# toandaominh1997/EfficientDet.Pytorch

Hardware: AMD Instinct MI355X
Metric: images/sec EfficientDet-D0 512px fwd+bwd (higher is better)
Workload: dtype f32_hf16x3_bwd_bf16x3

## Files before the change

efficientdet/pytorch_amd/_lib.py:

```python
import ctypes as C
import os

import torch

HERE = os.path.dirname(os.path.abspath(__file__))
LIB_PATH = os.environ.get('EFFDET_HIP_LIB') or os.path.join(os.path.dirname(os.path.abspath(__file__)), 'libeffdet_hip.so')
MAX_SEG = 5
MAX_CONV_SEG = 10
ABI_VERSION = 11
F32, BF16, F32_BF16X3, F32_SPLIT = 0, 1, 2, 3
F32_HSPLIT = 4
ACT_NONE, ACT_RELU, ACT_SWISH, ACT_SIGMOID = 0, 1, 2, 3
RES_NONE, RES_ADD, RES_RELU_MASK, RES_SWISH_GRAD = 0, 1, 2, 3
TUNE_IGEMM_BIG, TUNE_IGEMM_BIG_MIN_M, TUNE_SPLIT_PERS, TUNE_IGEMM_KORD, TUNE_SPLIT_KORD = 0, 1, 2, 3, 4
TUNE_ROWSLAB = 5

_ERR = {-1: 'EFFDET_EINVAL', -2: 'EFFDET_ELAUNCH', -3: 'EFFDET_EUNSUPPORTED'}


class Seg(C.Structure):
    _fields_ = [('H', C.c_int), ('W', C.c_int), ('Ho', C.c_int), ('Wo', C.c_int),
                ('in_off', C.c_longlong), ('in_bstride', C.c_longlong),
                ('out_off', C.c_longlong), ('out_bstride', C.c_longlong)]


class ConvDesc(C.Structure):
    _fields_ = [('x', C.c_void_p), ('w', C.c_void_p), ('y', C.c_void_p), ('z', C.c_void_p), ('res', C.c_void_p),
                ('scale', C.c_void_p), ('shift', C.c_void_p), ('rowscale', C.c_void_p),
                ('bc_scale', C.c_void_p), ('bc_shift', C.c_void_p),
                ('dtype', C.c_int), ('out_f32', C.c_int),
                ('B', C.c_int), ('Cin', C.c_int), ('Cout', C.c_int), ('KH', C.c_int), ('KW', C.c_int),
                ('stride', C.c_int), ('pad_t', C.c_int), ('pad_l', C.c_int),
                ('ldx', C.c_int), ('ldy', C.c_int), ('act', C.c_int), ('res_mode', C.c_int),
                ('nseg', C.c_int), ('seg', Seg * MAX_CONV_SEG), ('w_image_stride', C.c_longlong), ('y_split', C.c_void_p), ('range_flag', C.c_void_p),
                ('seg_w', C.c_void_p * MAX_CONV_SEG), ('seg_shift', C.c_void_p * MAX_CONV_SEG)]


class WgradDesc(C.Structure):
    _fields_ = [('x', C.c_void_p), ('dz', C.c_void_p), ('dw', C.c_void_p), ('dbias', C.c_void_p),
                ('dtype', C.c_int),
                ('B', C.c_int), ('Cin', C.c_int), ('Cout', C.c_int), ('KH', C.c_int), ('KW', C.c_int),
                ('stride', C.c_int), ('pad_t', C.c_int), ('pad_l', C.c_int),
                ('ldx', C.c_int), ('lddz', C.c_int), ('nseg', C.c_int), ('image_splits', C.c_int), ('seg', Seg * MAX_SEG)]


class PrepJob(C.Structure):
    _fields_ = [('a', C.c_void_p), ('b', C.c_void_p), ('c', C.c_void_p), ('d', C.c_void_p), ('out', C.c_void_p),
                ('kind', C.c_int), ('dtype', C.c_int), ('n0', C.c_int), ('n1', C.c_int), ('n2', C.c_int), ('n3', C.c_int),
                ('n4', C.c_int), ('eps', C.c_float)]


class UnpackJob(C.Structure):
    _fields_ = [(n, C.c_void_p) for n in ('g', 'scale', 'w_oihw', 'dw_oihw', 'wsum', 'dsum_part', 'mean', 'invstd', 'dgamma', 'dbeta',
                                          'dbias_out', 'slab_scale', 'slab_cscale')] + \
               [(n, C.c_int) for n in ('accumulate', 'Cout', 'Cin', 'KH', 'KW', 'Cin_pad', 'nslabs', 'slabs_per_scale')]


class SeParamJob(C.Structure):
    _fields_ = [(n, C.c_void_p) for n in ('du', 'dmid', 'sw', 'pool', 'dw1', 'db1', 'dw2', 'db2')] + \
               [('B', C.c_int), ('C', C.c_int), ('Cse', C.c_int), ('inv_hw', C.c_float)]


class DwUnpackJob(C.Structure):
    _fields_ = [(n, C.c_void_p) for n in ('g_kkc', 'scale', 'w_c1kk', 'dw_c1kk', 'wsum', 'dsum', 'mean', 'invstd', 'dgamma', 'dbeta')] + \
               [('C', C.c_int), ('kk', C.c_int)]


class _TailUnion(C.Union):
# ... 381 lines not shown
```

efficientdet/pytorch_amd/csrc/conv_igemm.hip:

```cpp
#include "common.h"
#include "../../../include/effdet_live_tiles.h"
#include "../../../include/effdet_needed_tiles.h"
#include "../../../include/effdet_unit_lists.h"
#include "../../../include/effdet_conv_plan.h"
#include "../../../include/effdet_gate_operand.h"
#include <stdlib.h>

#ifndef EFFDET_IGEMM_BIG_DEFAULT
#define EFFDET_IGEMM_BIG_DEFAULT 1
#endif

namespace {

struct SegD {
  int H, W, Ho, Wo, M, tile_start;
  long long in_off, in_bs, out_off, out_bs;
  unsigned x_bytes;
  long long w_off;
  long long sh_off;
};

struct ConvK {
  const void* x; const void* w; void* y; void* z; const void* res;
  const float* scale; const float* shift; const float* rowscale;
  const float* bc_scale; const float* bc_shift;
  int Cin, Cout, KW, stride, pad_t, pad_l;
  int ldx, ldy;
  int Kc;
  int cpt;
  int act, res_mode, out_f32, vec_ok;
  int out_split;
  int* range_flag;
  void* ysplit;
  int nseg, mtiles, ntiles;
  unsigned w_bytes;
  int kord;
  long long w_img_bytes;
  const unsigned char* live;
  int live_tile0;
  const unsigned char* needed;
  int needed_tile0;
  const unsigned char* uflags32; const int* units; const int* ucounts;
  long long g_in_off; unsigned g_x_bytes;
  const float* a_gate;
  int slab;
  int xld;
  SegD seg[EFFDET_MAX_CONV_SEG];
};

constexpr int BM = 128;

__host__ __device__ inline int slab_entries(int W) { return (BM / W) * (W + 2); }
__host__ __device__ inline bool slab_seg_ok(const SegD& s, int bn) {
  return (s.W & (s.W - 1)) == 0 && s.W >= (bn > 64 ? 8 : 16) && s.W <= 64 && s.Ho == s.H && s.Wo == s.W;
}
typedef float f32x16 __attribute__((ext_vector_type(16)));

template <typename T> struct Mma;
template <> struct Mma<bf16_t> {
  static __device__ __forceinline__ void run(const uint4& a, const uint4& b, f32x4& c) {
    c = __builtin_amdgcn_mfma_f32_16x16x32_bf16(__builtin_bit_cast(bf16x8, a), __builtin_bit_cast(bf16x8, b), c, 0, 0, 0);
  }
};
struct MmaH {
  static __device__ __forceinline__ void run(const uint4& a, const uint4& b, f32x4& c) {
    c = __builtin_amdgcn_mfma_f32_16x16x32_f16(__builtin_bit_cast(f16x8, a), __builtin_bit_cast(f16x8, b), c, 0, 0, 0);
  }
};
template <> struct Mma<float> {
  static __device__ __forceinline__ void run(const uint4& a, const uint4& b, f32x4& c) {
    c = __builtin_amdgcn_mfma_f32_16x16x4f32(__uint_as_float(a.x), __uint_as_float(b.x), c, 0, 0, 0);
    c = __builtin_amdgcn_mfma_f32_16x16x4f32(__uint_as_float(a.y), __uint_as_float(b.y), c, 0, 0, 0);
    c = __builtin_amdgcn_mfma_f32_16x16x4f32(__uint_as_float(a.z), __uint_as_float(b.z), c, 0, 0, 0);
    c = __builtin_amdgcn_mfma_f32_16x16x4f32(__uint_as_float(a.w), __uint_as_float(b.w), c, 0, 0, 0);
  }
};

template <typename T, int BN, int WAVES_N, int NWAVES, int SPLIT = 0, int NS = 2, int M32 = 0, int GATE = 0>
__global__ __launch_bounds__(NWAVES * 64, (SPLIT == 3 && NWAVES == 4) ? 3 : 1) void conv_igemm_kernel(const ConvK p) {
  static_assert(!SPLIT || sizeof(T) == 4, "bf16x3 splitting applies to fp32 storage");
  static_assert(!M32 || SPLIT == 2, "the 32x32x16 form is built for the split layout");
  static_assert(SPLIT != 3 || NS == 2, "f16x3: two stages");
  static_assert(NS == 2 || !M32, "deep staging is not built for the 32x32 tile loop");
  static_assert(!GATE || (SPLIT == 0 && sizeof(T) == 4), "the operand gate is built for the exact-fp32 form");
  constexpr int CE = Elem<T>::CE;
  constexpr int NTHREADS = NWAVES * 64;
  constexpr int WAVES_M = NWAVES / WAVES_N;
  constexpr int WTM = BM / WAVES_M, WTN = BN / WAVES_N;
  constexpr int MT = WTM / 16, NT = WTN / 16;
  constexpr int XLD = BM * 8;
  constexpr int WLD = BN * 8;
  constexpr int RSTEP = NTHREADS / 8;
  constexpr int XROWS = BM / RSTEP;
  constexpr int WROWS = (BN + RSTEP - 1) / RSTEP;

  constexpr bool SLABCAP = SPLIT >= 2 && NS == 2 && !M32;
  constexpr int SP = SLABCAP ? (160 + RSTEP - 1) / RSTEP : 1;
  static_assert(!SLABCAP || ((SP - 1) * RSTEP == 128 && WROWS * RSTEP == BN), "slab passes: 128 entries for every wave, the rest in the last pass");
  static_assert(!SLABCAP || MT <= 2, "slab fragments: fragment 1 is one uniform entry step from fragment 0");

  extern __shared__ __attribute__((aligned(16))) uint4 smem[];
  const int xld = SLABCAP ? p.xld : XLD;
  uint4* xs = SLABCAP ? smem + NS * WLD : smem;
  uint4* ws = SLABCAP ? smem : smem + NS * XLD;

  const int tid = threadIdx.x;
  const int lane = tid & 63, wave = tid >> 6;
  const int wm0 = (wave / WAVES_N) * WTM, wn0 = (wave % WAVES_N) * WTN;

  int tile = xcd_remap(blockIdx.x, gridDim.x);
  if constexpr (SPLIT == 2) {
    if (p.live) {
      const int b = blockIdx.x, whole = (p.mtiles >> 3) << 3;
      if (b < whole * p.ntiles) {
        const int i = b >> 3, j = i / p.ntiles;
        tile = (j * 8 + (b & 7)) * p.ntiles + (i - j * p.ntiles);
      } else tile = b;
    }
  }
  if constexpr (SPLIT == 3) {
    if (p.needed) {
      const int b = blockIdx.x, whole = (p.mtiles >> 3) << 3;
      if (b < whole * p.ntiles) {
        const int i = b >> 3, j = i / p.ntiles;
        tile = (j * 8 + (b & 7)) * p.ntiles + (i - j * p.ntiles);
      } else tile = b;
    }
  }
  const int mt = tile / p.ntiles, nt = tile - mt * p.ntiles;
  int si = 0;
#pragma unroll
  for (int s = 1; s < EFFDET_MAX_CONV_SEG; ++s)
    if (s < p.nseg && mt >= p.seg[s].tile_start) si = s;
  const SegD sg = p.seg[si];
  const int m_base = (mt - sg.tile_start) * BM;
  const int n_base = nt * BN;
  const int HoWo = sg.Ho * sg.Wo;
// ... 139 lines not shown
#pragma unroll
    for (int j = 0; j < WROWS; ++j) {
      if (wrow0 + RSTEP * j < BN)
        dma16_async(rw, ws_a + (unsigned)(buf * WLD + (wrow0 + RSTEP * j) * 8) * 16u, (kok && wok[j]) ? woff[j] + (unsigned)kq * 16u : EFFDET_OOB);
    }
    if constexpr (SPLIT != 1) {
      if (p.kord == 1) {
        const int taps = p.Kc / p.cpt;
        ++tapi;
        if (++kw == p.KW) { kw = 0; ++kh; }
        if (tapi == taps) { tapi = 0; kh = 0; kw = 0; cc += 8; }
        kq = (cc < p.cpt) ? tapi * p.cpt + cc : p.Kc;
        retap();
        return;
      }
    }
    kq += 8; cc += 8;
    if (cc < p.cpt) {
#pragma unroll
      for (int j = 0; j < XROWS; ++j) xcur[j] = (xcur[j] == EFFDET_OOB) ? EFFDET_OOB : xcur[j] + 128u;
    } else {
      while (cc >= p.cpt) { cc -= p.cpt; ++kw; if (kw == p.KW) { kw = 0; ++kh; } }
      retap();
    }
  };

  f32x4 acc[NT][MT];
#pragma unroll
  for (int a = 0; a < NT; ++a)
#pragma unroll
    for (int b = 0; b < MT; ++b) acc[a][b] = f32x4{0.f, 0.f, 0.f, 0.f};

  const int nk = (p.Kc + 7) >> 3;
  const int l15 = lane & 15, lq = lane >> 4, lsw = l15 >> 1;
  float* const gl = (float*)(smem + NS * (XLD + WLD));
  if constexpr (GATE) {
    const float* grow = p.a_gate + (long long)(m_base / HoWo) * p.Cin;
    for (int i = tid; i < nk * 32; i += NTHREADS) gl[i] = i < p.Cin ? grow[i] : 0.f;
  }
  auto load = [&](int buf, int s, uint4 (&wf)[NT], uint4 (&xf)[MT]) {
    const int ch = ((s * 4 + lq) ^ lsw);
#pragma unroll
    for (int a = 0; a < NT; ++a) wf[a] = ws[buf * WLD + (wn0 + a * 16 + l15) * 8 + ch];
#pragma unroll
    for (int b = 0; b < MT; ++b) xf[b] = xs[buf * XLD + (wm0 + b * 16 + l15) * 8 + ch];
  };
  auto mma = [&](const uint4 (&wf)[NT], const uint4 (&xf)[MT]) {
#pragma unroll
    for (int a = 0; a < NT; ++a)
#pragma unroll
      for (int b = 0; b < MT; ++b) Mma<T>::run(wf[a], xf[b], acc[a][b]);
  };
  constexpr int PPS = XROWS + WROWS;
  auto wait_tile = [&](int ahead) {
    if constexpr (NS == 2) { (void)ahead; dma_wait_all(); }
    else {
      if (NS >= 4 && ahead >= 2) asm volatile("s_waitcnt vmcnt(%0)" :: "n"(2 * PPS) : "memory");
      else if (ahead >= 1) asm volatile("s_waitcnt vmcnt(%0)" :: "n"(PPS) : "memory");
      else dma_wait_all();
    }
  };
  constexpr int NT32 = M32 ? WTN / 32 : 1, MT32 = M32 ? WTM / 32 : 1;
  f32x16 acc32[NT32][MT32];
  const int l31 = lane & 31, lh = lane >> 5;
  if constexpr (M32) {
    static_assert(WTN % 32 == 0 && WTM % 32 == 0, "32x32 MFMA tiles");
#pragma unroll
    for (int a = 0; a < NT32; ++a)
#pragma unroll
      for (int b = 0; b < MT32; ++b)
#pragma unroll
        for (int e = 0; e < 16; ++e) acc32[a][b][e] = 0.f;
    const int sw32 = (l31 >> 1) & 7;
    auto mm32 = [](const uint4& a, const uint4& b, f32x16& c) {
      c = __builtin_amdgcn_mfma_f32_32x32x16_bf16(__builtin_bit_cast(bf16x8, a), __builtin_bit_cast(bf16x8, b), c, 0, 0, 0);
    };
    auto kstep = [&](int buf) {
#pragma unroll
      for (int kk = 0; kk < 2; ++kk) {
        uint4 wh[NT32], wl[NT32], xh[MT32], xl[MT32];
        const int ch = ((2 * kk + lh) ^ sw32), cl = ((4 + 2 * kk + lh) ^ sw32);
#pragma unroll
        for (int a = 0; a < NT32; ++a) wh[a] = ws[buf * WLD + (wn0 + a * 32 + l31) * 8 + ch];
#pragma unroll
        for (int b = 0; b < MT32; ++b) xh[b] = xs[buf * XLD + (wm0 + b * 32 + l31) * 8 + ch];
#pragma unroll
        for (int b = 0; b < MT32; ++b) xl[b] = xs[buf * XLD + (wm0 + b * 32 + l31) * 8 + cl];
#pragma unroll
        for (int a = 0; a < NT32; ++a) wl[a] = ws[buf * WLD + (wn0 + a * 32 + l31) * 8 + cl];
#pragma unroll
        for (int t = 0; t < 3; ++t)
#pragma unroll
          for (int a = 0; a < NT32; ++a)
#pragma unroll
            for (int b = 0; b < MT32; ++b) mm32(t == 2 ? wl[a] : wh[a], t == 1 ? xl[b] : xh[b], acc32[a][b]);
      }
    };
    stage(0);
    if (nk > 1) stage(1);
    dma_wait_all();
    __syncthreads();
    for (int kt = 0; kt < nk; ++kt) {
      const int c = kt & 1;
      kstep(c);
      if (kt + 1 < nk) {
        dma_wait_all();
        __syncthreads();
        if (kt + 2 < nk) stage(c);
      }
    }
  } else if constexpr (SPLIT) {
    struct Frags { uint4 wh[NT], wl[NT], xh[MT], xl[MT]; };
    f32x4 acc2[SPLIT == 3 ? NT : 1][SPLIT == 3 ? MT : 1];
// ... 814 lines not shown
          const f32x4 xv = xt[cur][pl * C4 + k];
#pragma unroll
          for (int j = 0; j < 4; ++j) {
            const f32x2v xx = f32x2v{xv[j], xv[j]};
            a01 = __builtin_elementwise_fma(w01[4 * k + j], xx, a01);
            a23 = __builtin_elementwise_fma(w23[4 * k + j], xx, a23);
          }
        }
        f32x4 v = f32x4{a01[0], a01[1], a23[0], a23[1]} * sc + sh;
        if (p.z) *(f32x4*)((float*)p.z + o) = v;
        if (p.act == EFFDET_ACT_RELU) { for (int r = 0; r < 4; ++r) v[r] = relu_(v[r]); }
        else if (p.act == EFFDET_ACT_SWISH) { for (int r = 0; r < 4; ++r) v[r] = swishf_(v[r]); }
        else if (p.act == EFFDET_ACT_SIGMOID) { for (int r = 0; r < 4; ++r) v[r] = sigmoidf_(v[r]); }
        if (p.rowscale || p.bc_scale) {
          const int bi = m / HoWo;
          if (p.rowscale) v *= p.rowscale[bi];
          if (p.bc_scale) { const int bo = bi * p.Cout + n0; v = v * *(const f32x4*)(p.bc_scale + bo) + *(const f32x4*)(p.bc_shift + bo); }
        }
        if (p.res_mode == EFFDET_RES_ADD) { v += q; }
        else if (p.res_mode == EFFDET_RES_RELU_MASK) { for (int r = 0; r < 4; ++r) v[r] = relu_bwd_(q[r], v[r]); }
        else if (p.res_mode == EFFDET_RES_SWISH_GRAD) { for (int r = 0; r < 4; ++r) v[r] *= swish_gradf_(q[r]); }
        *(f32x4*)((float*)p.y + o) = v;
      }
    }
    if (tile + 1 < ntile) sstore(cur ^ 1);
    __syncthreads();
  }
}

static bool pw_eligible(const effdet_conv_t* p) {
  static const int on = getenv("EFFDET_CONV_PW") ? atoi(getenv("EFFDET_CONV_PW")) : 1;
  if (!on || p->dtype != EFFDET_F32 || p->out_f32 || p->nseg != 1 || p->KH != 1 || p->KW != 1 || p->stride != 1 || p->pad_t || p->pad_l) return false;
  if ((p->Cin != 16 && p->Cin != 24) || p->Cout % 4 || p->Cout < 32 || p->Cout > 1024) return false;
  const effdet_seg_t& g = p->seg[0];
  if (g.H != g.Ho || g.W != g.Wo || p->ldx != p->Cin || p->ldy != p->Cout) return false;
  if (g.in_bstride != (long long)g.H * g.W * p->ldx || g.out_bstride != (long long)g.Ho * g.Wo * p->ldy) return false;
  if (g.in_off % 4 || g.out_off % 4) return false;
  return (long long)p->B * g.H * g.W >= 65536;
}

struct ConvPlan {
  int id;
  ConvK k;
  int (*launch)(const ConvPlan&, hipStream_t);
  unsigned grid;
  size_t lds;
  int pw_G, pw_NPS, pw_ppw;
  int form, pers;
  int tile_m, tile_n, stages, threads, m32;
  int ksteps;
  int gate;
};

static int g_tuning[EFFDET_TUNE_COUNT] = {-1, 16384, -1, 1, -1, -1};
static bool rowslab_on() {
  if (g_tuning[EFFDET_TUNE_ROWSLAB] < 0) g_tuning[EFFDET_TUNE_ROWSLAB] = getenv("EFFDET_ROWSLAB") ? atoi(getenv("EFFDET_ROWSLAB")) : 1;
  return g_tuning[EFFDET_TUNE_ROWSLAB] != 0;
}

template <typename T, int BN, int WAVES_N, int NWAVES, int SPLIT, int NS, int M32, int GATE>
int launch_igemm(const ConvPlan& c, hipStream_t st) {
  if (c.lds > 48 * 1024) EFFDET_SET_MAX_LDS((conv_igemm_kernel<T, BN, WAVES_N, NWAVES, SPLIT, NS, M32, GATE>), c.lds);
  hipLaunchKernelGGL((conv_igemm_kernel<T, BN, WAVES_N, NWAVES, SPLIT, NS, M32, GATE>), dim3(c.grid), dim3(NWAVES * 64), c.lds, st, c.k);
  EFFDET_CHECK_LAUNCH();
  return EFFDET_OK;
}
template <typename T, int BN, int WAVES_N, int NWAVES, int SPLIT = 0, int NS = 2, int M32 = 0, int GATE = 0>
int use_igemm(ConvPlan& c, int id) {
  c.k.ntiles = (c.k.Cout + BN - 1) / BN;
  c.grid = (unsigned)(c.k.mtiles * c.k.ntiles);
  c.k.slab = 0; c.k.xld = BM * 8;
  if constexpr (SPLIT >= 2 && NS == 2 && !M32) {
    const ConvK& k = c.k;
    if (rowslab_on() && k.kord == 1 && k.KW == 3 && k.Kc == 9 * k.cpt && k.stride == 1 && k.pad_t == 1 && k.pad_l == 1) {
      int ent = 0;
      for (int s = 0; s < k.nseg; ++s)
        if (slab_seg_ok(k.seg[s], BN) && ((slab_entries(k.seg[s].W) + 7) & ~7) > ent) ent = (slab_entries(k.seg[s].W) + 7) & ~7;
      if (ent) { c.k.slab = 1; c.k.xld = (ent > BM ? ent : BM) * 8; }
    }
  }
  c.lds = (size_t)NS * (c.k.xld + BN * 8) * sizeof(uint4);
  if (GATE) c.lds += (size_t)((c.k.Kc + 7) >> 3) * 32 * sizeof(float);
  c.gate = GATE;
  c.launch = launch_igemm<T, BN, WAVES_N, NWAVES, SPLIT, NS, M32, GATE>;
  static_assert(EFFDET_CONV_FORM_PLAIN == 0 && EFFDET_CONV_FORM_BF16X3 == 1 && EFFDET_CONV_FORM_SPLIT == 2 && EFFDET_CONV_FORM_HSPLIT == 3,
                "the kernel's SPLIT parameter is the public form code");
  c.form = SPLIT; c.pers = 0; c.tile_m = BM; c.tile_n = BN; c.stages = NS; c.threads = NWAVES * 64; c.m32 = M32;
  c.ksteps = (c.k.Kc + 7) >> 3;
  return c.id = id;
}

template <int WM, int WN, int NS, int X3>
int launch_pers(const ConvPlan& c, hipStream_t st) {
  EFFDET_SET_MAX_LDS((conv_igemm_pers_kernel<WM, WN, NS, X3>), c.lds);
  static unsigned ncu = 0;
  if (ncu == 0) { int dev = 0; hipDeviceProp_t pr; ncu = (hipGetDevice(&dev) == hipSuccess && hipGetDeviceProperties(&pr, dev) == hipSuccess) ? pr.multiProcessorCount : 256; }
  const unsigned grid = c.grid < ncu ? c.grid : ncu;
  hipLaunchKernelGGL((conv_igemm_pers_kernel<WM, WN, NS, X3>), dim3(grid), dim3(WM * WN * 64), c.lds, st, c.k);
  EFFDET_CHECK_LAUNCH();
  return EFFDET_OK;
}
template <int WM, int WN, int NS, int X3 = 0>
int use_pers(ConvPlan& c, int id) {
  constexpr int TM = 64 * WM, TN = 64 * WN;
  ConvK& k = c.k;
  k.mtiles = 0;
  for (int s = 0; s < k.nseg; ++s) { k.seg[s].tile_start = k.mtiles; k.mtiles += (k.seg[s].M + TM - 1) / TM; }
  k.ntiles = (k.Cout + TN - 1) / TN;
  if (X3) {
    k.ldx *= 2;
    for (int s = 0; s < k.nseg; ++s) { k.seg[s].in_off *= 2; k.seg[s].in_bs *= 2; }
  }
  c.grid = (unsigned)(k.mtiles * k.ntiles);
  c.lds = (size_t)NS * (TM + TN) * 128;
  c.launch = launch_pers<WM, WN, NS, X3>;
  c.form = X3 ? EFFDET_CONV_FORM_SPLIT : EFFDET_CONV_FORM_PLAIN; c.pers = 1; c.tile_m = TM; c.tile_n = TN; c.stages = NS; c.threads = WM * WN * 64; c.m32 = 1;
  c.ksteps = (k.Kc / k.cpt) * (k.cpt >> 3);
  return c.id = id;
}
static int use_big(ConvPlan& c, int id) {
  switch (id) {
    case 10 + 442: return use_pers<4, 4, 2>(c, id);
    case 10 + 242: return use_pers<2, 4, 2>(c, id);
    case 10 + 243: return use_pers<2, 4, 3>(c, id);
    case 10 + 4220: return use_pers<4, 2, 2>(c, id);
    default: return use_pers<4, 2, 3>(c, id);
  }
}

template <int CIN>
int launch_pw(const ConvPlan& c, hipStream_t st) {
  hipLaunchKernelGGL(conv_pw_f32_kernel<CIN>, dim3(c.grid), dim3(256), 0, st, c.k, c.k.seg[0].M, c.pw_G, c.pw_NPS, c.pw_ppw);
  EFFDET_CHECK_LAUNCH();
  return EFFDET_OK;
}
static int use_pw(ConvPlan& c) {
  c.pw_G = c.k.Cout / 4; c.pw_NPS = 256 / c.pw_G; c.pw_ppw = 1024;
  c.grid = (unsigned)((c.k.seg[0].M + c.pw_ppw - 1) / c.pw_ppw);
  c.lds = 0;
  c.launch = c.k.Cin == 16 ? launch_pw<16> : launch_pw<24>;
  c.form = EFFDET_CONV_FORM_SKINNY; c.pers = 0; c.tile_m = 64; c.tile_n = c.k.Cout; c.stages = 2; c.threads = 256; c.m32 = 0;
  c.k.mtiles = (int)c.grid; c.k.ntiles = 1; c.ksteps = 1;
  return c.id = 20;
}

static int big_variant() {
  if (g_tuning[EFFDET_TUNE_IGEMM_BIG] < 0)
    g_tuning[EFFDET_TUNE_IGEMM_BIG] = getenv("EFFDET_IGEMM_BIG") ? atoi(getenv("EFFDET_IGEMM_BIG")) : EFFDET_IGEMM_BIG_DEFAULT;
  return g_tuning[EFFDET_TUNE_IGEMM_BIG];
}

template <typename T, int SPLIT, int GATE = 0>
int use_tile(ConvPlan& c, int bt) {
  const ConvK& k = c.k;
  const int id = bt + (SPLIT ? 4 : 0), bn = 128 >> bt;
  const long long tiles = (long long)k.mtiles * ((k.Cout + bn - 1) / bn);
  static const int deep_env = getenv("EFFDET_IGEMM_DEEP") ? atoi(getenv("EFFDET_IGEMM_DEEP")) : 2;
  if ((SPLIT ? deep_env >= 2 : deep_env >= 1) && tiles <= 256 && k.Kc >= 6 * 8) {
    static const int narrow = getenv("EFFDET_IGEMM_NARROW") ? atoi(getenv("EFFDET_IGEMM_NARROW")) : 128;
    static const int narrow_k = getenv("EFFDET_IGEMM_NARROW_K") ? atoi(getenv("EFFDET_IGEMM_NARROW_K")) : 16;
    if (narrow && bt <= 1 && tiles <= narrow && k.Kc >= narrow_k * 8) return use_igemm<T, 32, 1, 4, SPLIT, 4, 0, GATE>(c, id);
    if (bt == 0) return use_igemm<T, 128, 2, 8, SPLIT, 4, 0, GATE>(c, id);
    if (bt == 1) return use_igemm<T, 64, 1, 4, SPLIT, 4, 0, GATE>(c, id);
  }
  switch (bt) {
    case 0: return use_igemm<T, 128, 2, 8, SPLIT, 2, 0, GATE>(c, id);
    case 1: return use_igemm<T, 64, 1, 4, SPLIT, 2, 0, GATE>(c, id);
    case 2: return use_igemm<T, 32, 1, 4, SPLIT, 2, 0, GATE>(c, id);
    default: return use_igemm<T, 16, 1, 4, SPLIT, 2, 0, GATE>(c, id);
  }
}

}

extern "C" int effdet_tuning_set(int key, int value) {
  if (key < 0 || key >= EFFDET_TUNE_COUNT) return EFFDET_EINVAL;
  (void)big_variant();
  const int old = g_tuning[key];
  g_tuning[key] = value;
  return old;
}

static int plan_conv(const effdet_conv_t* p, ConvPlan& c, const float* a_gate = nullptr, int a_act = EFFDET_ACT_NONE) {
  ConvK& k = c.k;
  c.gate = 0;
  if (!p || !p->x || !p->w || !p->y) return EFFDET_EINVAL;
  if (p->nseg < 1 || p->nseg > EFFDET_MAX_CONV_SEG) return EFFDET_EINVAL;
  if (p->dtype != EFFDET_F32 && p->dtype != EFFDET_BF16 && p->dtype != EFFDET_F32_BF16X3 && p->dtype != EFFDET_F32_SPLIT && p->dtype != EFFDET_F32_HSPLIT) return EFFDET_EINVAL;
  const int ce = p->dtype == EFFDET_BF16 ? 8 : 4;
  if (p->Cin % ce || p->ldx % ce || p->KH < 1 || p->KW < 1 || p->stride < 1) return EFFDET_EUNSUPPORTED;
  if (p->res_mode != EFFDET_RES_NONE && !p->res) return EFFDET_EINVAL;
  const bool hfmt = p->dtype == EFFDET_F32_HSPLIT;
  const bool splitfmt = p->dtype == EFFDET_F32_SPLIT || hfmt;
  if (hfmt && (p->res_mode != EFFDET_RES_NONE || p->scale || p->bc_scale || p->rowscale || p->w_image_stride || (p->KH * p->KW * p->Cin) % 32)) return EFFDET_EUNSUPPORTED;
  if (splitfmt) {
    if (p->Cin % 32 || p->ldx % 32 || p->z) return EFFDET_EUNSUPPORTED;
    if (p->out_f32 ? (p->res_mode != EFFDET_RES_NONE && p->res_mode != EFFDET_RES_ADD)
                   : (p->Cout % 32 || p->ldy % 32 || (p->res_mode != EFFDET_RES_NONE && p->res_mode != EFFDET_RES_RELU_MASK))) return EFFDET_EUNSUPPORTED;
    for (int s = 0; s < p->nseg; ++s) {
      if (p->seg[s].in_off % 32 || p->seg[s].in_bstride % 32) return EFFDET_EUNSUPPORTED;
      if (!p->out_f32 && (p->seg[s].out_off % 32 || p->seg[s].out_bstride % 32)) return EFFDET_EUNSUPPORTED;
    }
  } else if (p->out_f32 && (p->z || p->res_mode != EFFDET_RES_NONE)) return EFFDET_EUNSUPPORTED;
  if (p->y_split) {
    if ((p->dtype != EFFDET_F32 && !hfmt) || p->out_f32 || p->res_mode != EFFDET_RES_NONE || p->Cout % 32 || p->ldy % 32) return EFFDET_EUNSUPPORTED;
    for (int s = 0; s < p->nseg; ++s)
      if (p->seg[s].out_off % 32 || p->seg[s].out_bstride % 32) return EFFDET_EUNSUPPORTED;
  }
  k.x = p->x; k.w = p->w; k.y = p->y; k.z = p->z; k.res = p->res; k.ysplit = p->y_split; k.range_flag = hfmt ? p->range_flag : nullptr;
  k.scale = p->scale; k.shift = p->shift; k.rowscale = p->rowscale;
  k.bc_scale = p->bc_scale; k.bc_shift = p->bc_shift;
  if ((p->bc_scale != nullptr) != (p->bc_shift != nullptr)) return EFFDET_EINVAL;
  k.Cin = p->Cin; k.Cout = p->Cout; k.KW = p->KW; k.stride = p->stride; k.pad_t = p->pad_t; k.pad_l = p->pad_l;
  k.ldx = p->ldx; k.ldy = p->ldy;
  k.cpt = p->Cin / ce; k.Kc = p->KH * p->KW * k.cpt;
  k.act = p->act; k.res_mode = p->res_mode; k.out_f32 = p->out_f32; k.kord = g_tuning[EFFDET_TUNE_IGEMM_KORD];
  k.out_split = (splitfmt && !p->out_f32) ? 1 : 0;
  if (splitfmt) {
    if (g_tuning[EFFDET_TUNE_SPLIT_KORD] < 0) g_tuning[EFFDET_TUNE_SPLIT_KORD] = getenv("EFFDET_SPLIT_KORD") ? atoi(getenv("EFFDET_SPLIT_KORD")) : 1;
    const int kv = g_tuning[EFFDET_TUNE_SPLIT_KORD];
    k.kord = ((kv == 1 || (kv == 2 && p->Cout <= 64)) && k.cpt % 8 == 0) ? 1 : 0;
  }
  k.nseg = p->nseg;
  k.w_img_bytes = p->w_image_stride;
  k.live = nullptr; k.live_tile0 = 0;
  k.needed = nullptr; k.needed_tile0 = 0;
  k.uflags32 = nullptr; k.units = nullptr; k.ucounts = nullptr; k.g_in_off = 0; k.g_x_bytes = 0;
  k.a_gate = a_gate;
  k.slab = 0; k.xld = BM * 8;
  if (a_gate) {
    if (a_act != EFFDET_ACT_NONE && a_act != EFFDET_ACT_SWISH) return EFFDET_EINVAL;
    if (p->dtype != EFFDET_F32 || p->KH != 1 || p->KW != 1 || p->stride != 1 || p->pad_t || p->pad_l || p->nseg != 1 || p->w_image_stride ||
        p->seg[0].H != p->seg[0].Ho || p->seg[0].W != p->seg[0].Wo || (p->seg[0].Ho * p->seg[0].Wo) % BM || ((size_t)a_gate & 3)) return EFFDET_EUNSUPPORTED;
  }
  if (p->w_image_stride) {
    if (p->w_image_stride < 0 || (p->w_image_stride & 15) || p->nseg != 1 || splitfmt || (p->seg[0].Ho * p->seg[0].Wo) % BM) return EFFDET_EUNSUPPORTED;
  }
  int tiles = 0;
  bool per_seg = false;
  bool vec = (p->ldy % 4 == 0) && (p->Cout % 4 == 0);
  for (int s = 0; s < p->nseg; ++s) {
    const effdet_seg_t& g = p->seg[s];
    SegD& d = k.seg[s];
    d.H = g.H; d.W = g.W; d.Ho = g.Ho; d.Wo = g.Wo;
    d.M = p->B * g.Ho * g.Wo;
    d.tile_start = tiles;
    d.in_off = g.in_off; d.in_bs = g.in_bstride; d.out_off = g.out_off; d.out_bs = g.out_bstride;
    d.w_off = p->seg_w[s] ? (long long)((const char*)p->seg_w[s] - (const char*)p->w) : 0ll;
    d.sh_off = p->seg_shift[s] ? (long long)(p->seg_shift[s] - p->shift) : 0ll;
    if (p->seg_w[s] || p->seg_shift[s]) per_seg = true;
    if ((p->seg_shift[s] && !p->shift) || (d.w_off & 15)) return EFFDET_EINVAL;
    if (d.M <= 0) return EFFDET_EINVAL;
    if (g.in_off % ce || g.in_bstride % ce) return EFFDET_EUNSUPPORTED;
    if (g.out_off % 4 || g.out_bstride % 4) vec = false;
    tiles += (d.M + BM - 1) / BM;
  }
  for (int s = p->nseg; s < EFFDET_MAX_CONV_SEG; ++s) { k.seg[s] = k.seg[0]; k.seg[s].tile_start = 0x7fffffff; }
  k.mtiles = tiles; k.vec_ok = vec ? 1 : 0;
  if (per_seg && (p->w_image_stride || p->scale)) return EFFDET_EUNSUPPORTED;
  const long long es = p->dtype == EFFDET_BF16 ? 2 : 4;
  for (int s = 0; s < p->nseg; ++s) {
    const effdet_seg_t& g = p->seg[s];
    const long long e = ((long long)(p->B - 1) * g.in_bstride + ((long long)(g.H - 1) * g.W + (g.W - 1)) * p->ldx + p->Cin) * es;
    if (e >= 0xFFFF0000LL) return EFFDET_EUNSUPPORTED;
    k.seg[s].x_bytes = (unsigned)e;
  }
  const long long wb = (long long)p->Cout * k.Kc * 16;
  if (wb >= 0xFFFF0000LL) return EFFDET_EUNSUPPORTED;
  k.w_bytes = (unsigned)wb;
  if (hfmt) {
    k.scale = (const float*)((const char*)p->w + wb);
    return p->Cout > 64 ? use_igemm<float, 128, 2, 8, 3>(c, 30) : use_igemm<float, 64, 1, 4, 3>(c, 31);
  }
  long long mtot = 0;
  bool fits = true;
  for (int s = 0; s < p->nseg; ++s) {
    mtot += k.seg[s].M;
    if ((long long)k.seg[s].x_bytes + 2LL * ((long long)p->KH * p->seg[s].W + p->KW) * p->ldx * es >= 0x70000000LL) fits = false;
  }
  if (p->dtype == EFFDET_BF16 && !per_seg && !p->bc_scale && !p->w_image_stride && p->Cin % 64 == 0 && p->KH * p->KW <= 32 && p->Cout >= 128 && big_variant() != 0 && wb < 0x40000000LL &&
      fits && mtot >= g_tuning[EFFDET_TUNE_IGEMM_BIG_MIN_M]) {
    const int v = big_variant();
    if (v == 1) {
      const long long K = (long long)k.Kc * 8;
      if (p->Cout >= 192 && mtot >= 65536 && ((p->res_mode == EFFDET_RES_NONE && K >= 2304) || K >= 4608)) return use_big(c, 10 + 442);
    } else if (v == 442 || v == 242 || v == 243 || v == 423) {
      return use_big(c, 10 + ((p->Cout > 128 || v == 423) ? v : (v == 243 ? 4230 : 4220)));
    }
  }
  if (a_gate) {
    if (per_seg) return EFFDET_EUNSUPPORTED;
    k.kord = 0;
    const int gbt = k.Cout > 64 ? 0 : k.Cout > 32 ? 1 : k.Cout > 16 ? 2 : 3;
    return a_act == EFFDET_ACT_SWISH ? use_tile<float, 0, 2>(c, gbt) : use_tile<float, 0, 1>(c, gbt);
  }
  if (!per_seg && !p->w_image_stride && !p->y_split && pw_eligible(p)) return use_pw(c);
  const int bt = k.Cout > 64 ? 0 : k.Cout > 32 ? 1 : k.Cout > 16 ? 2 : 3;
  if (p->dtype == EFFDET_F32_BF16X3) {
    if (k.Kc % 8) return EFFDET_EUNSUPPORTED;
    k.kord = 0;
    return use_tile<float, 1>(c, bt);
  }
  if (p->dtype == EFFDET_F32_SPLIT) {
    if (g_tuning[EFFDET_TUNE_SPLIT_PERS] < 0) g_tuning[EFFDET_TUNE_SPLIT_PERS] = getenv("EFFDET_SPLIT_PERS") ? atoi(getenv("EFFDET_SPLIT_PERS")) : 2;
    if (g_tuning[EFFDET_TUNE_SPLIT_PERS] > 0 && !per_seg && !p->bc_scale && p->KH * p->KW <= 32 && p->Cout >= 192 && wb < 0x40000000LL) {
      const int pv = g_tuning[EFFDET_TUNE_SPLIT_PERS];
      const bool pick = pv == 1 || (pv == 2 && p->res_mode == EFFDET_RES_NONE) || (pv == 3 && p->res_mode != EFFDET_RES_NONE);
      if (pick && fits && mtot >= g_tuning[EFFDET_TUNE_IGEMM_BIG_MIN_M] && (long long)k.Kc * 4 >= 1152) return use_pers<4, 4, 2, 1>(c, 10000 + 442);
// ... 123 lines not shown
```

efficientdet/pytorch_amd/ops.py:

```python
import ctypes as C
import os
import threading

import numpy as np
import torch

from . import _lib as L
from ._lib import (ACT_NONE, ACT_RELU, ACT_SIGMOID, ACT_SWISH, RES_ADD, RES_NONE,
                   RES_RELU_MASK, RES_SWISH_GRAD)


class LaunchProfile:

    def __init__(self):
        self.records = []

    def summary(self):
        torch.cuda.synchronize()
        out = {}
        for name, flops, e0, e1, _, nbytes in self.records:
            d = out.setdefault(name, {'launches': 0, 'flops': 0.0, 'ms': 0.0, 'bytes': 0.0})
            d['launches'] += 1; d['flops'] += flops; d['ms'] += e0.elapsed_time(e1); d['bytes'] += nbytes
        return out

# ... 58 lines not shown
    return t


def clear_range_flag(device):
    range_flag(device).fill_(0)


def check_range_flag(device, what='f16x3'):
    t = range_flag(device)
    if int(t.item()) != 0:
        t.zero_()
        raise FloatingPointError('%s: an activation of the RetinaHead / BiFPN left the range of the fp16 operand split (|x| >= 65520 or NaN); '
                                 "the outputs of this call are not valid -- use f32_arith='f32_bwd_bf16x3' or 'f32' for this model" % what)


class backward_scope:

    def __init__(self, prep, arith):
        self.prep, self.arith = prep, arith

    def __enter__(self):
        self.old = (F32_ARITH, F32_ARITH_BWD, F32_ARITH_HEAD)
        set_prep(self.prep); set_f32_arith(self.arith)
        return self

    def __exit__(self, et, ev, tb):
        global F32_ARITH, F32_ARITH_BWD, F32_ARITH_HEAD
        F32_ARITH, F32_ARITH_BWD, F32_ARITH_HEAD = self.old
        return False


def _mma_dtype_code(dtype, K=None, N=None):
    code = L.dtype_code(dtype)
    if code != L.F32 or F32_ARITH != 'bf16x3':
        return code
    if K is not None and (K % 32 or K < 256 or N < 32):
        return code
    return L.F32_BF16X3


def _igemm_symbol(dtype, desc):
    kid = int(L.lib().effdet_conv2d_kernel(C.byref(desc)))
    if kid in (30, 31):
        return 'conv_igemm_kernel<hsplit,%d,f16x3>' % (128, 64)[kid - 30]
    if kid >= 10000:
        return 'conv_igemm_pers_kernel<split,bf16x3>'
    if kid == 20:
        return 'conv_pw_f32_kernel'
    if kid >= 10:
        v = str(kid - 10)
        return 'conv_igemm_pers_kernel<%s,%s,%s>' % (v[0], v[1], v[2])
    if kid in (8, 9):
        return 'conv_igemm_kernel<split,%d,bf16x3>' % (128, 64)[kid - 8]
    if 4 <= kid < 8:
        return 'conv_igemm_kernel<f32,%d,bf16x3>' % (128, 64, 32, 16)[kid - 4]
    return 'conv_igemm_kernel<%s,%d>' % ('bf16' if dtype == torch.bfloat16 else 'f32', (128, 64, 32, 16)[max(kid, 0)])


class Map:
    __slots__ = ('t', 'B', 'H', 'W', 'C', 'ld', 'bstride', 'off')

    def __init__(self, t, B, H, W, C, ld=None, bstride=None, off=0):
        self.t, self.B, self.H, self.W, self.C = t, B, H, W, C
        self.ld = C if ld is None else ld
        self.bstride = H * W * self.ld if bstride is None else bstride
        self.off = off

    @staticmethod
    def new(B, H, W, C, dtype, device, zero=False):
        f = torch.zeros if zero else torch.empty
        return Map(f((B, H, W, C), dtype=dtype, device=device), B, H, W, C)

    @staticmethod
    def of(t):
        assert t.dim() == 4 and t.is_contiguous()
        return Map(t, t.shape[0], t.shape[1], t.shape[2], t.shape[3])

    @property
    def dtype(self):
        return self.t.dtype

    def addr(self):
        return self.t.data_ptr() + self.off * self.t.element_size()

    def tensor(self):
        assert self.ld == self.C and self.bstride == self.H * self.W * self.C and self.off == 0
        return self.t.view(self.B, self.H, self.W, self.C)


def _segs(desc, xs, ys, base_x, base_y, isz_x, isz_y):
    desc.nseg = len(xs)
    for i, (x, y) in enumerate(zip(xs, ys)):
        s = desc.seg[i]
        s.H, s.W, s.Ho, s.Wo = x.H, x.W, y.H, y.W
        dx = x.addr() - base_x
        dy = y.addr() - base_y
        assert dx % isz_x == 0 and dy % isz_y == 0
        s.in_off, s.in_bstride = dx // isz_x, x.bstride
        s.out_off, s.out_bstride = dy // isz_y, y.bstride


PREP_PACK0, PREP_PACK1, PREP_BNFOLD, PREP_DWPACK = 0, 1, 2, 3

_PARAM_GENERATION = 0


# ... 2403 lines not shown
```

include/effdet_hip.h:

```cpp
#ifndef EFFDET_HIP_H
#define EFFDET_HIP_H
#ifdef __cplusplus
extern "C" {
#endif

typedef void* effdet_stream_t;

enum { EFFDET_OK = 0, EFFDET_EINVAL = -1, EFFDET_ELAUNCH = -2, EFFDET_EUNSUPPORTED = -3 };
enum { EFFDET_F32 = 0, EFFDET_BF16 = 1,
       EFFDET_F32_BF16X3 = 2,
       EFFDET_F32_SPLIT = 3,
       EFFDET_F32_HSPLIT = 4 };
enum { EFFDET_ACT_NONE = 0, EFFDET_ACT_RELU = 1, EFFDET_ACT_SWISH = 2, EFFDET_ACT_SIGMOID = 3 };
enum { EFFDET_RES_NONE = 0, EFFDET_RES_ADD = 1, EFFDET_RES_RELU_MASK = 2, EFFDET_RES_SWISH_GRAD = 3 };

#define EFFDET_MAX_SEG 5
#define EFFDET_MAX_CONV_SEG 10

typedef struct {
  int H, W, Ho, Wo;
  long long in_off, in_bstride, out_off, out_bstride;
} effdet_seg_t;

typedef struct {
  const void* x; const void* w; void* y; void* z; const void* res;
  const float* scale; const float* shift;
  const float* rowscale;
  const float* bc_scale; const float* bc_shift;
  int dtype, out_f32;
  int B, Cin, Cout, KH, KW, stride, pad_t, pad_l;
  int ldx, ldy;
  int act, res_mode;
  int nseg;
  effdet_seg_t seg[EFFDET_MAX_CONV_SEG];
  long long w_image_stride;
  void* y_split;
  int* range_flag;
  const void* seg_w[EFFDET_MAX_CONV_SEG];
  const float* seg_shift[EFFDET_MAX_CONV_SEG];
} effdet_conv_t;
int effdet_conv2d(const effdet_conv_t* p, effdet_stream_t stream);
int effdet_scale_pack_weight(const float* w, const float* gate, void* out, int dtype, int B, int Cout, int Cin, effdet_stream_t stream);

int effdet_conv2d_kernel(const effdet_conv_t* p);

enum { EFFDET_TUNE_IGEMM_BIG = 0, EFFDET_TUNE_IGEMM_BIG_MIN_M = 1,
       EFFDET_TUNE_SPLIT_PERS = 2 ,
       EFFDET_TUNE_IGEMM_KORD = 3 ,
       EFFDET_TUNE_SPLIT_KORD = 4 ,
       EFFDET_TUNE_ROWSLAB = 5 ,
       EFFDET_TUNE_COUNT = 6 };
int effdet_tuning_set(int key, int value);

typedef struct {
  const void* x; const void* dz; float* dw; float* dbias;
  int dtype;
  int B, Cin, Cout, KH, KW, stride, pad_t, pad_l;
  int ldx, lddz;
  int nseg;
  int image_splits;
  effdet_seg_t seg[EFFDET_MAX_SEG];
} effdet_wgrad_t;
long long effdet_conv2d_wgrad_workspace_bytes(const effdet_wgrad_t* p);
int effdet_conv2d_wgrad_splits(const effdet_wgrad_t* p);
int effdet_conv2d_wgrad_seg_slabs(const effdet_wgrad_t* p, int* first, int* count);
int effdet_conv2d_wgrad_kernel(const effdet_wgrad_t* p);
int effdet_conv2d_wgrad(const effdet_wgrad_t* p, void* workspace, long long workspace_bytes, effdet_stream_t stream);

int effdet_pack_conv_weight(const float* w_oihw, const float* scale, void* out, int dtype, int mode,
                            int Cout, int Cin, int KH, int KW, int Cin_pad, effdet_stream_t stream);
int effdet_unpack_conv_wgrad(const float* g, const float* scale, const float* w_oihw, float* dw_oihw,
                             float* wsum, int accumulate, int Cout, int Cin, int KH, int KW, int Cin_pad, int nslabs,
                             const float* dbias_part, float* dbias_out, const float* slab_scale, int slabs_per_scale,
                             effdet_stream_t stream);
int effdet_unpack_conv_wgrad_bn(const float* g, const float* scale, const float* w_oihw, float* dw_oihw, const float* dsum_part,
                                const float* mean, const float* invstd, float* dgamma, float* dbeta, int Cout, int Cin,
                                int KH, int KW, int Cin_pad, int nslabs, const float* slab_scale, int slabs_per_scale,
                                effdet_stream_t stream);

typedef struct {
  const float* g; const float* scale; const float* w_oihw; float* dw_oihw; float* wsum;
  const float* dsum_part; const float* mean; const float* invstd; float* dgamma; float* dbeta; float* dbias_out;
  const float* slab_scale;
  const float* slab_cscale;
  int accumulate, Cout, Cin, KH, KW, Cin_pad, nslabs, slabs_per_scale;
} effdet_unpack_job_t;
int effdet_unpack_conv_wgrad_batch(const effdet_unpack_job_t* jobs, int njobs, effdet_stream_t stream);

enum { EFFDET_TAIL_UNPACK = 0, EFFDET_TAIL_SE_PARAMS = 1, EFFDET_TAIL_DW_UNPACK = 2 };
typedef struct {
  const float* du; const float* dmid; const float* sw; const float* pool;
  float* dw1; float* db1; float* dw2; float* db2;
  int B, C, Cse; float inv_hw;
} effdet_se_param_job_t;
typedef struct {
  const float* g_kkc; const float* scale; const float* w_c1kk; float* dw_c1kk; float* wsum;
  const float* dsum; const float* mean; const float* invstd; float* dgamma; float* dbeta;
  int C, kk;
} effdet_dw_unpack_job_t;
typedef struct {
  int kind;
  union { effdet_unpack_job_t conv; effdet_se_param_job_t se; effdet_dw_unpack_job_t dw; } u;
} effdet_tail_job_t;
int effdet_backward_tail(const effdet_tail_job_t* jobs, int njobs, effdet_stream_t stream);
// ... 257 lines not shown
```

Baseline: 1442.

## Add short 32-row pixel tile igemm variant for small narrow convolutions

Makes the igemm kernel's pixel-tile height BM a template parameter. For exact-fp32 and register-split bf16x3 convolutions with few workgroups and no per-image weights, the planner now picks a 32-pixel by 32-channel tile with 2x2 waves and 8-stage staging. This spreads small low-resolution layers over more workgroups to fill the GPU, and the per-stage vmcnt wait becomes a generic recursion. The cost is more tile overhead and weight reloads per pixel. Only fp32 and f32_bf16x3 forms qualify, so layers running in the f16x3 split form are unaffected.

Result: faster. 1461, median of 6 (+1.3%).

```diff
diff --git a/efficientdet/pytorch_amd/_lib.py b/efficientdet/pytorch_amd/_lib.py
--- a/efficientdet/pytorch_amd/_lib.py
+++ b/efficientdet/pytorch_amd/_lib.py
@@ -14,6 +14,7 @@
 RES_NONE, RES_ADD, RES_RELU_MASK, RES_SWISH_GRAD = 0, 1, 2, 3
 TUNE_IGEMM_BIG, TUNE_IGEMM_BIG_MIN_M, TUNE_SPLIT_PERS, TUNE_IGEMM_KORD, TUNE_SPLIT_KORD = 0, 1, 2, 3, 4
 TUNE_ROWSLAB = 5
+TUNE_SHORT_TILE = 7
 
 _ERR = {-1: 'EFFDET_EINVAL', -2: 'EFFDET_ELAUNCH', -3: 'EFFDET_EUNSUPPORTED'}
 
diff --git a/efficientdet/pytorch_amd/csrc/conv_igemm.hip b/efficientdet/pytorch_amd/csrc/conv_igemm.hip
--- a/efficientdet/pytorch_amd/csrc/conv_igemm.hip
+++ b/efficientdet/pytorch_amd/csrc/conv_igemm.hip
@@ -48,13 +48,22 @@
   SegD seg[EFFDET_MAX_CONV_SEG];
 };
 
-constexpr int BM = 128;
-
-__host__ __device__ inline int slab_entries(int W) { return (BM / W) * (W + 2); }
+constexpr int BM128 = 128;
+
+__host__ __device__ inline int slab_entries(int W) { return (BM128 / W) * (W + 2); }
 __host__ __device__ inline bool slab_seg_ok(const SegD& s, int bn) {
   return (s.W & (s.W - 1)) == 0 && s.W >= (bn > 64 ? 8 : 16) && s.W <= 64 && s.Ho == s.H && s.Wo == s.W;
 }
 typedef float f32x16 __attribute__((ext_vector_type(16)));
+
+template <int PPS, int A>
+__device__ __forceinline__ void wait_ahead(int ahead) {
+  if constexpr (A == 0) { (void)ahead; dma_wait_all(); }
+  else {
+    if (ahead >= A) asm volatile("s_waitcnt vmcnt(%0)" :: "n"(A * PPS) : "memory");
+    else wait_ahead<PPS, A - 1>(ahead);
+  }
+}
 
 template <typename T> struct Mma;
 template <> struct Mma<bf16_t> {
@@ -76,13 +85,15 @@
   }
 };
 
-template <typename T, int BN, int WAVES_N, int NWAVES, int SPLIT = 0, int NS = 2, int M32 = 0, int GATE = 0>
+template <typename T, int BN, int WAVES_N, int NWAVES, int SPLIT = 0, int NS = 2, int M32 = 0, int GATE = 0, int BM = BM128>
 __global__ __launch_bounds__(NWAVES * 64, (SPLIT == 3 && NWAVES == 4) ? 3 : 1) void conv_igemm_kernel(const ConvK p) {
   static_assert(!SPLIT || sizeof(T) == 4, "bf16x3 splitting applies to fp32 storage");
   static_assert(!M32 || SPLIT == 2, "the 32x32x16 form is built for the split layout");
   static_assert(SPLIT != 3 || NS == 2, "f16x3: two stages");
   static_assert(NS == 2 || !M32, "deep staging is not built for the 32x32 tile loop");
   static_assert(!GATE || (SPLIT == 0 && sizeof(T) == 4), "the operand gate is built for the exact-fp32 form");
+  static_assert(BM == BM128 || (sizeof(T) == 4 && SPLIT <= 1 && !M32 && !GATE && NS > 2), "short pixel tiles: exact fp32 / register-split bf16x3, deep staging");
+  static_assert(BM % (NWAVES * 8) == 0 && BM % (16 * (NWAVES / WAVES_N)) == 0, "whole DMA passes and whole 16-row MFMA tiles per wave");
   constexpr int CE = Elem<T>::CE;
   constexpr int NTHREADS = NWAVES * 64;
   constexpr int WAVES_M = NWAVES / WAVES_N;
@@ -328,13 +339,10 @@
       for (int b = 0; b < MT; ++b) Mma<T>::run(wf[a], xf[b], acc[a][b]);
   };
   constexpr int PPS = XROWS + WROWS;
+  static_assert(NS == 2 || (BN >= RSTEP && (NS - 2) * PPS <= 63), "deep staging: the same pieces in every wave, a count s_waitcnt vmcnt can hold");
   auto wait_tile = [&](int ahead) {
     if constexpr (NS == 2) { (void)ahead; dma_wait_all(); }
-    else {
-      if (NS >= 4 && ahead >= 2) asm volatile("s_waitcnt vmcnt(%0)" :: "n"(2 * PPS) : "memory");
-      else if (ahead >= 1) asm volatile("s_waitcnt vmcnt(%0)" :: "n"(PPS) : "memory");
-      else dma_wait_all();
-    }
+    else wait_ahead<PPS, NS - 2>(ahead);
   };
   constexpr int NT32 = M32 ? WTN / 32 : 1, MT32 = M32 ? WTM / 32 : 1;
   f32x16 acc32[NT32][MT32];
@@ -1255,21 +1263,25 @@
   int gate;
 };
 
-static int g_tuning[EFFDET_TUNE_COUNT] = {-1, 16384, -1, 1, -1, -1};
+static int g_tuning[EFFDET_TUNE_COUNT] = {-1, 16384, -1, 1, -1, -1, 0 , 1};
 static bool rowslab_on() {
   if (g_tuning[EFFDET_TUNE_ROWSLAB] < 0) g_tuning[EFFDET_TUNE_ROWSLAB] = getenv("EFFDET_ROWSLAB") ? atoi(getenv("EFFDET_ROWSLAB")) : 1;
   return g_tuning[EFFDET_TUNE_ROWSLAB] != 0;
 }
 
-template <typename T, int BN, int WAVES_N, int NWAVES, int SPLIT, int NS, int M32, int GATE>
+template <typename T, int BN, int WAVES_N, int NWAVES, int SPLIT, int NS, int M32, int GATE, int BM>
 int launch_igemm(const ConvPlan& c, hipStream_t st) {
-  if (c.lds > 48 * 1024) EFFDET_SET_MAX_LDS((conv_igemm_kernel<T, BN, WAVES_N, NWAVES, SPLIT, NS, M32, GATE>), c.lds);
-  hipLaunchKernelGGL((conv_igemm_kernel<T, BN, WAVES_N, NWAVES, SPLIT, NS, M32, GATE>), dim3(c.grid), dim3(NWAVES * 64), c.lds, st, c.k);
+  if (c.lds > 48 * 1024) EFFDET_SET_MAX_LDS((conv_igemm_kernel<T, BN, WAVES_N, NWAVES, SPLIT, NS, M32, GATE, BM>), c.lds);
+  hipLaunchKernelGGL((conv_igemm_kernel<T, BN, WAVES_N, NWAVES, SPLIT, NS, M32, GATE, BM>), dim3(c.grid), dim3(NWAVES * 64), c.lds, st, c.k);
   EFFDET_CHECK_LAUNCH();
   return EFFDET_OK;
 }
-template <typename T, int BN, int WAVES_N, int NWAVES, int SPLIT = 0, int NS = 2, int M32 = 0, int GATE = 0>
+template <typename T, int BN, int WAVES_N, int NWAVES, int SPLIT = 0, int NS = 2, int M32 = 0, int GATE = 0, int BM = BM128>
 int use_igemm(ConvPlan& c, int id) {
+  if constexpr (BM != BM128) {
+    c.k.mtiles = 0;
+    for (int s = 0; s < c.k.nseg; ++s) { c.k.seg[s].tile_start = c.k.mtiles; c.k.mtiles += (c.k.seg[s].M + BM - 1) / BM; }
+  }
   c.k.ntiles = (c.k.Cout + BN - 1) / BN;
   c.grid = (unsigned)(c.k.mtiles * c.k.ntiles);
   c.k.slab = 0; c.k.xld = BM * 8;
@@ -1279,13 +1291,13 @@
       int ent = 0;
       for (int s = 0; s < k.nseg; ++s)
         if (slab_seg_ok(k.seg[s], BN) && ((slab_entries(k.seg[s].W) + 7) & ~7) > ent) ent = (slab_entries(k.seg[s].W) + 7) & ~7;
-      if (ent) { c.k.slab = 1; c.k.xld = (ent > BM ? ent : BM) * 8; }
+      if (ent) { c.k.slab = 1; c.k.xld = (ent > BM128 ? ent : BM128) * 8; }
     }
   }
   c.lds = (size_t)NS * (c.k.xld + BN * 8) * sizeof(uint4);
   if (GATE) c.lds += (size_t)((c.k.Kc + 7) >> 3) * 32 * sizeof(float);
   c.gate = GATE;
-  c.launch = launch_igemm<T, BN, WAVES_N, NWAVES, SPLIT, NS, M32, GATE>;
+  c.launch = launch_igemm<T, BN, WAVES_N, NWAVES, SPLIT, NS, M32, GATE, BM>;
   static_assert(EFFDET_CONV_FORM_PLAIN == 0 && EFFDET_CONV_FORM_BF16X3 == 1 && EFFDET_CONV_FORM_SPLIT == 2 && EFFDET_CONV_FORM_HSPLIT == 3,
                 "the kernel's SPLIT parameter is the public form code");
   c.form = SPLIT; c.pers = 0; c.tile_m = BM; c.tile_n = BN; c.stages = NS; c.threads = NWAVES * 64; c.m32 = M32;
@@ -1362,7 +1374,15 @@
   if ((SPLIT ? deep_env >= 2 : deep_env >= 1) && tiles <= 256 && k.Kc >= 6 * 8) {
     static const int narrow = getenv("EFFDET_IGEMM_NARROW") ? atoi(getenv("EFFDET_IGEMM_NARROW")) : 128;
     static const int narrow_k = getenv("EFFDET_IGEMM_NARROW_K") ? atoi(getenv("EFFDET_IGEMM_NARROW_K")) : 16;
-    if (narrow && bt <= 1 && tiles <= narrow && k.Kc >= narrow_k * 8) return use_igemm<T, 32, 1, 4, SPLIT, 4, 0, GATE>(c, id);
+    if (narrow && bt <= 1 && tiles <= narrow && k.Kc >= narrow_k * 8) {
+      if constexpr (sizeof(T) == 4 && SPLIT <= 1 && !GATE) {
+        constexpr int SHORT_MAX_WG = 96, SHORT_MAX_WG_2N = 128;
+        const int nwg = k.mtiles * ((k.Cout + 31) / 32);
+        if (g_tuning[EFFDET_TUNE_SHORT_TILE] != 0 && !k.w_img_bytes && (nwg <= SHORT_MAX_WG || (k.Cout <= 64 && nwg <= SHORT_MAX_WG_2N)))
+          return use_igemm<T, 32, 2, 4, SPLIT, 8, 0, 0, 32>(c, id);
+      }
+      return use_igemm<T, 32, 1, 4, SPLIT, 4, 0, GATE>(c, id);
+    }
     if (bt == 0) return use_igemm<T, 128, 2, 8, SPLIT, 4, 0, GATE>(c, id);
     if (bt == 1) return use_igemm<T, 64, 1, 4, SPLIT, 4, 0, GATE>(c, id);
   }
@@ -1377,7 +1397,7 @@
 }
 
 extern "C" int effdet_tuning_set(int key, int value) {
-  if (key < 0 || key >= EFFDET_TUNE_COUNT) return EFFDET_EINVAL;
+  if (key < 0 || key >= EFFDET_TUNE_COUNT || key == EFFDET_TUNE_ROWSLAB + 1) return EFFDET_EINVAL;
   (void)big_variant();
   const int old = g_tuning[key];
   g_tuning[key] = value;
@@ -1430,14 +1450,14 @@
   k.needed = nullptr; k.needed_tile0 = 0;
   k.uflags32 = nullptr; k.units = nullptr; k.ucounts = nullptr; k.g_in_off = 0; k.g_x_bytes = 0;
   k.a_gate = a_gate;
-  k.slab = 0; k.xld = BM * 8;
+  k.slab = 0; k.xld = BM128 * 8;
   if (a_gate) {
     if (a_act != EFFDET_ACT_NONE && a_act != EFFDET_ACT_SWISH) return EFFDET_EINVAL;
     if (p->dtype != EFFDET_F32 || p->KH != 1 || p->KW != 1 || p->stride != 1 || p->pad_t || p->pad_l || p->nseg != 1 || p->w_image_stride ||
-        p->seg[0].H != p->seg[0].Ho || p->seg[0].W != p->seg[0].Wo || (p->seg[0].Ho * p->seg[0].Wo) % BM || ((size_t)a_gate & 3)) return EFFDET_EUNSUPPORTED;
+        p->seg[0].H != p->seg[0].Ho || p->seg[0].W != p->seg[0].Wo || (p->seg[0].Ho * p->seg[0].Wo) % BM128 || ((size_t)a_gate & 3)) return EFFDET_EUNSUPPORTED;
   }
   if (p->w_image_stride) {
-    if (p->w_image_stride < 0 || (p->w_image_stride & 15) || p->nseg != 1 || splitfmt || (p->seg[0].Ho * p->seg[0].Wo) % BM) return EFFDET_EUNSUPPORTED;
+    if (p->w_image_stride < 0 || (p->w_image_stride & 15) || p->nseg != 1 || splitfmt || (p->seg[0].Ho * p->seg[0].Wo) % BM128) return EFFDET_EUNSUPPORTED;
   }
   int tiles = 0;
   bool per_seg = false;
@@ -1456,7 +1476,7 @@
     if (d.M <= 0) return EFFDET_EINVAL;
     if (g.in_off % ce || g.in_bstride % ce) return EFFDET_EUNSUPPORTED;
     if (g.out_off % 4 || g.out_bstride % 4) vec = false;
-    tiles += (d.M + BM - 1) / BM;
+    tiles += (d.M + BM128 - 1) / BM128;
   }
   for (int s = p->nseg; s < EFFDET_MAX_CONV_SEG; ++s) { k.seg[s] = k.seg[0]; k.seg[s].tile_start = 0x7fffffff; }
   k.mtiles = tiles; k.vec_ok = vec ? 1 : 0;
diff --git a/efficientdet/pytorch_amd/ops.py b/efficientdet/pytorch_amd/ops.py
--- a/efficientdet/pytorch_amd/ops.py
+++ b/efficientdet/pytorch_amd/ops.py
@@ -134,6 +134,10 @@
         return 'conv_igemm_pers_kernel<%s,%s,%s>' % (v[0], v[1], v[2])
     if kid in (8, 9):
         return 'conv_igemm_kernel<split,%d,bf16x3>' % (128, 64)[kid - 8]
+    if 0 <= kid < 8 and dtype == torch.float32:
+        info = L.ConvPlanInfo()
+        if int(L.require('effdet_conv2d_plan_info').effdet_conv2d_plan_info(C.byref(desc), C.byref(info))) == kid and info.tile_m < 128:
+            return 'conv_igemm_kernel<f32,%d%s,short%d>' % (info.tile_n, ',bf16x3' if kid >= 4 else '', info.tile_m)
     if 4 <= kid < 8:
         return 'conv_igemm_kernel<f32,%d,bf16x3>' % (128, 64, 32, 16)[kid - 4]
     return 'conv_igemm_kernel<%s,%d>' % ('bf16' if dtype == torch.bfloat16 else 'f32', (128, 64, 32, 16)[max(kid, 0)])
diff --git a/include/effdet_hip.h b/include/effdet_hip.h
--- a/include/effdet_hip.h
+++ b/include/effdet_hip.h
@@ -49,7 +49,8 @@
        EFFDET_TUNE_IGEMM_KORD = 3 ,
        EFFDET_TUNE_SPLIT_KORD = 4 ,
        EFFDET_TUNE_ROWSLAB = 5 ,
-       EFFDET_TUNE_COUNT = 6 };
+       EFFDET_TUNE_SHORT_TILE = 7 ,
+       EFFDET_TUNE_COUNT = 8 };
 int effdet_tuning_set(int key, int value);
 
 typedef struct {
```
